# PalamaraLab/FastSMC

Measured on NVIDIA B200. Metric: hmm_pair_sites_per_s, higher is better.
Workload: dtype f32

## Files before the change

fastsmc_b200/csrc/decode_fast.cuh:

```cuda
#pragma once

#include "decode_kernels.cuh"

namespace fsmc
{

constexpr int kMaxParamStates = 160;

struct FastModel {
  DeviceModel base;
  float colRatios[kMaxParamStates];
  float expTimes[kMaxParamStates];
  float prior[kMaxParamStates];
};

__device__ __forceinline__ uint32_t smemPtr(const void* p)
{
  return static_cast<uint32_t>(__cvta_generic_to_shared(p));
}
__device__ __forceinline__ void mbarInit(uint64_t* bar, const uint32_t count)
{
  asm volatile("mbarrier.init.shared::cta.b64 [%0], %1;" ::"r"(smemPtr(bar)), "r"(count) : "memory");
}
__device__ __forceinline__ void mbarExpectTx(uint64_t* bar, const uint32_t bytes)
// ... 248 lines not shown
          const float2 t = __fmul2_rn(pk(f4(u4, 2 * jp), f4(u4, 2 * jp + 1)), xx);
          const float au0 = au;
          const float au1 = fmaf(colRatios[k], au0, t.x);
          au = fmaf(colRatios[k1], au1, t.y);
          const float2 tt = __ffma2_rn(pk(f4(d4, 2 * jp), f4(d4, 2 * jp + 1)), xx, pk(au0, au1));
          const float2 w = __fmul2_rn(pk(f4(e4, 2 * jp), f4(e4, 2 * jp + 1)),
                                      __ffma2_rn(pk(f4(b4, 2 * jp), f4(b4, 2 * jp + 1)), pk(y[k], y[k1]), tt));
          y[k] = w.x;
          y[k1] = w.y;
        } else if (k < S) {
          y[k] = f4(e4, 2 * jp) * fmaf(f4(d4, 2 * jp), x[k], au);
        }
      }
    }
    {
      const int ql = QM - 1 - i;
      const float4 e4 = E[ql], b4 = Br[ql];
#pragma unroll
      for (int jp = 1; jp >= 0; --jp) {
        const int k = 4 * ql + 2 * jp, k1 = k + 1;
        const float s1 = run;
        const float s0 = s1 + x[k1];
        run = s0 + x[k];
        const float2 w = __fmul2_rn(pk(f4(e4, 2 * jp), f4(e4, 2 * jp + 1)),
                                    __ffma2_rn(pk(f4(b4, 2 * jp), f4(b4, 2 * jp + 1)), pk(s0, s1), pk(y[k], y[k1])));
        y[k] = w.x;
        y[k1] = w.y;
      }
    }
  }
  return run;
}

template <int S>
__device__ __forceinline__ void backwardStepFolded(const float (&x)[S], float (&y)[S], const float* row, const int cls)
{
  constexpr int SQ = (S + 3) / 4, Spad = SQ * 4, QM = (SQ + 1) / 2;
  static_assert(4 * QM < S - 1, "the lower half lies below the last state");
  const float4* UsE = reinterpret_cast<const float4*>(row + cls * Spad);
  const float4* DE = reinterpret_cast<const float4*>(row + (3 + cls) * Spad);
  const float4* BE = reinterpret_cast<const float4*>(row + (6 + cls) * Spad);
  const float4* Rr = reinterpret_cast<const float4*>(row + 9 * Spad);
  float bu = 0.f, bl = 0.f;
  float above = 0.f;
#pragma unroll
  for (int i = 0; i < QM; ++i) {
    const int qu = SQ - 1 - i;
    if (qu >= QM) {
      const float4 u4 = UsE[qu], r4 = Rr[qu];
#pragma unroll
      for (int jp = 1; jp >= 0; --jp) {
        const int k = 4 * qu + 2 * jp, k1 = k + 1;
        if (k1 < S) {
          const float2 t = __fmul2_rn(pk(f4(u4, 2 * jp), f4(u4, 2 * jp + 1)), pk(x[k], x[k1]));
          if (k1 == S - 1) {
            y[k1] = 0.f;
          } else {
            bu = fmaf(f4(r4, 2 * jp + 1), bu, above);
            y[k1] = bu;
          }
          bu = fmaf(f4(r4, 2 * jp), bu, t.y);
          y[k] = bu;
          above = t.x;
        } else if (k < S) {
          above = f4(u4, 2 * jp) * x[k];
          if (k == S - 1) {
            y[k] = 0.f;
          } else {
            bu = fmaf(f4(r4, 2 * jp), bu, above);
            y[k] = bu;
          }
        }
      }
    }
    {
      const int ql = i;
      const float4 d4 = DE[ql], b4 = BE[ql];
#pragma unroll
      for (int jp = 0; jp < 2; ++jp) {
        const int k = 4 * ql + 2 * jp, k1 = k + 1;
        const float bl0 = bl;
        const float bl1 = fmaf(f4(b4, 2 * jp), x[k], bl0);
        bl = fmaf(f4(b4, 2 * jp + 1), x[k1], bl1);
        const float2 w = __ffma2_rn(pk(f4(d4, 2 * jp), f4(d4, 2 * jp + 1)), pk(x[k], x[k1]), pk(bl0, bl1));
        y[k] = w.x;
        y[k1] = w.y;
      }
    }
  }
#pragma unroll
  for (int i = 0; i < QM; ++i) {
    {
      const int ql = QM - 1 - i;
      const float4 u4 = UsE[ql], r4 = Rr[ql];
#pragma unroll
      for (int jp = 1; jp >= 0; --jp) {
        const int k = 4 * ql + 2 * jp, k1 = k + 1;
        const float2 t = __fmul2_rn(pk(f4(u4, 2 * jp), f4(u4, 2 * jp + 1)), pk(x[k], x[k1]));
        const float b1 = fmaf(f4(r4, 2 * jp + 1), bu, above);
        const float b0 = fmaf(f4(r4, 2 * jp), b1, t.y);
        bu = b0;
        above = t.x;
        const float2 w = __fadd2_rn(pk(y[k], y[k1]), pk(b0, b1));
        y[k] = w.x;
        y[k1] = w.y;
      }
    }
    const int qu = QM + i;
    if (qu < SQ) {
      const float4 d4 = DE[qu], b4 = BE[qu];
#pragma unroll
      for (int jp = 0; jp < 2; ++jp) {
        const int k = 4 * qu + 2 * jp, k1 = k + 1;
        if (k1 < S) {
          const float bl0 = bl;
          const float bl1 = fmaf(f4(b4, 2 * jp), x[k], bl0);
          bl = fmaf(f4(b4, 2 * jp + 1), x[k1], bl1);
          const float2 w = __fadd2_rn(__ffma2_rn(pk(f4(d4, 2 * jp), f4(d4, 2 * jp + 1)), pk(x[k], x[k1]), pk(bl0, bl1)),
                                      pk(y[k], y[k1]));
          y[k] = w.x;
          y[k1] = w.y;
        } else if (k < S) {
          y[k] = fmaf(f4(d4, 2 * jp), x[k], bl) + y[k];
        }
      }
    }
  }
}

static __device__ __noinline__ int emitSparseItems(SparseItem* items, float* itemAlpha, unsigned long long* itemCount,
                                            const long long capacity, const bool pred, const uint32_t pair, const int block,
                                            const int first, const int last, int chain, const float4* alphaStart,
                                            const int lane, const int SQ)
{
  const unsigned mask = __ballot_sync(kFull, pred);
  if (!mask) {
    return chain;
  }
  unsigned long long base = 0;
  if (lane == 0) {
    base = atomicAdd(itemCount, static_cast<unsigned long long>(__popc(mask)));
  }
  base = __shfl_sync(kFull, base, 0);
  if (pred) {
    const long long slot = static_cast<long long>(base) + __popc(mask & ((1u << lane) - 1u));
    if (slot < capacity) {
      items[slot] = SparseItem{pair, block, first, last, chain};
      float4* dst = reinterpret_cast<float4*>(itemAlpha + static_cast<size_t>(slot) * SQ * 4);
      for (int q = 0; q < SQ; ++q) {
        dst[q] = alphaStart[q * 32 + lane];
      }
    }
    chain = static_cast<int>(slot);
  }
  return chain;
}

constexpr int kNarrowMaxQuads = 4;
constexpr int kNarrowGroup = 4;

template <int S_T, int RQ, int G> struct NarrowSlot {
  static constexpr int SQ = (S_T + 3) / 4, Spad = SQ * 4;
  static constexpr uint32_t kCoefBytes = kBwdArrays * Spad * 4;
  static constexpr uint32_t kRecBytes = RQ * 32 * 16;
  static constexpr uint32_t kBytes = G * kCoefBytes + (G + 1) * kRecBytes;
};

template <int S_T, int RQ, int G, int DEPTH, int THREADS, int MIN_BLOCKS, int SPARSE_V = 0>
__global__ void __launch_bounds__(THREADS, MIN_BLOCKS) decodeNarrowKernel(const FastModel fm, const DecodeArgs args)
{
  constexpr bool SPARSE = (SPARSE_V & 1) != 0;
  constexpr bool kSkipFwd = (SPARSE_V & 2) != 0, kSkipBwd = (SPARSE_V & 4) != 0;
  constexpr int kGroupUnroll = (SPARSE_V & 64) ? G / 2 : 1;
  constexpr bool kSkipAlpha = (SPARSE_V & 8) != 0, kSkipBoundaryItems = (SPARSE_V & 16) != 0, kSkipRunItems = (SPARSE_V & 32) != 0;
  constexpr int S = S_T;
  constexpr int SQ = (S + 3) / 4;
  constexpr int Spad = SQ * 4;
  constexpr int NR = 4 * RQ - 1;
  using Slot = NarrowSlot<S_T, RQ, G>;
  constexpr uint32_t kRecBytes = Slot::kRecBytes;
  constexpr uint32_t kCoefBytes = Slot::kCoefBytes;
  constexpr size_t kRecFloats = static_cast<size_t>(RQ) * 32 * 4;
  constexpr size_t kRowFloats = static_cast<size_t>(kRowArrays) * Spad;
  constexpr uint32_t kRowBytes = static_cast<uint32_t>(kRowFloats) * 4;
  constexpr size_t kBwdFloats = static_cast<size_t>(kBwdArrays) * Spad;
  constexpr int kWarps = THREADS / 32;
  constexpr size_t kWarpBytes = static_cast<size_t>(DEPTH) * Slot::kBytes;
  static_assert(S >= 4 * kNarrowMaxQuads && RQ >= 1 && RQ <= kNarrowMaxQuads, "record quads index the state vector");
  static_assert(G % 2 == 0, "the two state vectors swap roles every step");

  extern __shared__ __align__(128) unsigned char smemRaw[];
  const DeviceModel m = fm.base;
  const int lane = threadIdx.x & 31;
  const int warp = threadIdx.x >> 5;
  unsigned char* mine = smemRaw + static_cast<size_t>(warp) * kWarpBytes;
  uint64_t* bars = reinterpret_cast<uint64_t*>(smemRaw + static_cast<size_t>(kWarps) * kWarpBytes) + warp * DEPTH;
  auto coefArea = [&](const int slot) { return reinterpret_cast<float*>(mine + static_cast<size_t>(slot) * Slot::kBytes); };
  auto recArea = [&](const int slot) {
    return reinterpret_cast<float4*>(mine + static_cast<size_t>(slot) * Slot::kBytes + static_cast<size_t>(G) * kCoefBytes);
  };
  if (lane == 0) {
    for (int i = 0; i < DEPTH; ++i) {
      mbarInit(&bars[i], 1);
    }
    asm volatile("fence.mbarrier_init.release.cluster;" ::: "memory");
  }
  __syncwarp();
  uint32_t parity = 0;

  const unsigned flags = args.flags;
  const bool wantSeg = flags & FSMC_CALL_SEGMENTS;
  const bool wantAge = !SPARSE && (flags & FSMC_SEG_AGE) && wantSeg;
  const int sT = m.stateThreshold;
  const long long warpGlobal = static_cast<long long>(blockIdx.x) * kWarps + warp;
  float* slab = args.scratch + warpGlobal * args.scratchPerWarp;
  constexpr size_t kVecFloats = static_cast<size_t>(SQ) * 32 * 4;
  const int ckShift = SPARSE ? args.ckptShift : 0;
  const int ckMask = (1 << ckShift) - 1;
  float4* alphaStart = SPARSE ? reinterpret_cast<float4*>(args.alphaScratch + warpGlobal * kVecFloats) : nullptr;

  for (;;) {
    unsigned long long t = 0;
    if (lane == 0) {
      t = atomicAdd(args.tileCounter, 1ull);
    }
    t = __shfl_sync(kFull, t, 0);
    if (static_cast<long long>(t) >= args.numTiles) {
      break;
    }
    const int tile = args.order ? args.order[t] : static_cast<int>(t);
    const int nPairs = args.tilePairs[tile];
    const int from = args.tileFrom[tile];
    const int len = args.tileTo[tile] - from;
    const int scanFrom = wantSeg ? args.tileScanFrom[tile] : 0;
    const int scanTo = wantSeg ? args.tileScanTo[tile] : 0;
    const bool laneActive = lane < nPairs;
    const int srcLane = laneActive ? lane : nPairs - 1;
    const uint32_t pair = static_cast<uint32_t>(tile) * 32u + static_cast<uint32_t>(lane);
    PairBits bits;
    bits.a = m.haps + static_cast<size_t>(args.hapA[static_cast<size_t>(tile) * 32 + srcLane]) * m.wordsPerHap;
    bits.b = m.haps + static_cast<size_t>(args.hapB[static_cast<size_t>(tile) * 32 + srcLane]) * m.wordsPerHap;
    const float* rowBase = m.siteRows + static_cast<size_t>(from) * kRowFloats;
    const long long ckptSlot0 = SPARSE ? args.tileCkptBase[tile] : 0;
    auto storeVector = [&](const float (&v)[S], float4* dst) {
#pragma unroll
      for (int q = 0; q < SQ; ++q) {
        dst[q * 32 + lane] = make_float4(v[4 * q], 4 * q + 1 < S ? v[4 * q + 1] : 0.f, 4 * q + 2 < S ? v[4 * q + 2] : 0.f,
                                         4 * q + 3 < S ? v[4 * q + 3] : 0.f);
      }
    };
    auto storeCheckpoint = [&](const float (&v)[S], const int p) {
      storeVector(v, reinterpret_cast<float4*>(args.ckptBeta + static_cast<size_t>(ckptSlot0 + (p >> ckShift)) * kVecFloats));
    };

    float a[S], c[S];
    float acc[NR];
#pragma unroll
    for (int k = 0; k < NR; ++k) {
      acc[k] = 0.f;
    }

    auto stageRecord = [&](const float (&v)[S], float4* out, const float divisor) {
#pragma unroll
      for (int q = 0; q < RQ; ++q) {
        float w[4];
#pragma unroll
        for (int i = 0; i < 4; ++i) {
          const int k = 4 * q + i;
          w[i] = k == NR ? divisor : (k < sT ? v[k] : 0.f);
        }
        out[q * 32 + lane] = make_float4(w[0], w[1], w[2], w[3]);
      }
    };

    {
      const int steps = len - 1;
      const int first = SPARSE ? min(steps, (len % G) ? (len % G) : G) : G;
      const int nGroups = steps <= 0 ? 0 : 1 + (max(steps - first, 0) + G - 1) / G;
      auto groupBegin = [&](const int g) { return g == 0 ? 0 : first + (g - 1) * G; };
      auto prefetch = [&](const int g) {
        if (lane == 0) {
          const int j0 = groupBegin(g), j1 = min(steps, j0 + (g == 0 ? first : G));
          const int slot = g % DEPTH;
          const uint32_t bytes = static_cast<uint32_t>(j1 - j0) * kCoefBytes;
          mbarExpectTx(&bars[slot], bytes);
          bulkLoad(coefArea(slot), m.bwdRows + static_cast<size_t>(from + len - j1) * kBwdFloats, bytes, &bars[slot]);
        }
      };
      for (int g = 0; g < DEPTH && g < nGroups; ++g) {
        prefetch(g);
      }
#pragma unroll
      for (int k = 0; k < S; ++k) {
        a[k] = 1.f;
      }
      if constexpr (SPARSE) {
        storeCheckpoint(a, len - 1);
      }
      if (nGroups == 0) {
        stageRecord(a, recArea(0), 1.0f);
        fenceProxyAsync();
        __syncwarp();
        if (lane == 0) {
          bulkStore(slab, recArea(0), kRecBytes);
          bulkCommit();
        }
      }
      for (int g = 0; g < nGroups; ++g) {
        const int slot = g % DEPTH;
        const int j0 = groupBegin(g);
        const int n = min(g == 0 ? first : G, steps - j0);
        const float* coef = coefArea(slot);
        float4* stage = recArea(slot);
        if constexpr (SPARSE && !kSkipBwd) {
          if (g > 0 && ((len - 1 - j0) & ckMask) == ckMask) {
            storeCheckpoint(a, len - 1 - j0);
          }
        }
        if (lane == 0) {
          bulkWaitRead<DEPTH - 1>();
        }
        mbarWait(&bars[slot], (parity >> slot) & 1u);
        parity ^= 1u << slot;
        __syncwarp();
        if (g == 0) {
          stageRecord(a, stage + static_cast<size_t>(n) * RQ * 32, 1.0f);
        }
        auto step = [&](const int i, float (&x)[S], float (&y)[S], const bool rescale) {
          const int p = len - 2 - (j0 + i);
          const int cls = bits.cls(from + p + 1);
          backwardStepFolded<S>(x, y, coef + static_cast<size_t>(n - 1 - i) * kBwdFloats, cls);
          float divisor = 1.0f;
          if (rescale) {
            divisor = sumStates<S>(y);
            scaleStates<S>(y, 1.0f / divisor);
          }
          stageRecord(y, stage + static_cast<size_t>(n - 1 - i) * RQ * 32, divisor);
        };
#pragma unroll(kGroupUnroll)
        for (int i = 0; i < G; i += 2) {
          if (i < n) {
            step(i, a, c, false);
          }
          if (i + 1 < n) {
            step(i + 1, c, a, i + 1 == G - 1);
          }
        }
        fenceProxyAsync();
        __syncwarp();
        if (lane == 0) {
          const int j1 = j0 + n;
          bulkStore(slab + static_cast<size_t>(len - 1 - j1) * kRecFloats, stage,
                    static_cast<uint32_t>(n + (g == 0 ? 1 : 0)) * kRecBytes);
          bulkCommit();
        }
        if (g + DEPTH < nGroups) {
          prefetch(g + DEPTH);
        }
        if (SPARSE && g == 0 && (n & 1)) {
#pragma unroll
          for (int k = 0; k < S; ++k) {
            a[k] = c[k];
          }
        }
      }
      const int rest = SPARSE ? max(steps - first, 0) : steps;
      if (rest & 1) {
      } else {
#pragma unroll
        for (int k = 0; k < S; ++k) {
          c[k] = a[k];
        }
      }
      if (lane == 0) {
        bulkWaitAll<0>();
      }
      __syncwarp();
    }

    {
      const int nGroups = (len + G - 1) / G;
      auto prefetch = [&](const int g) {
        if (lane == 0) {
          const int p0 = g * G;
          const uint32_t n = static_cast<uint32_t>(min(G, len - p0));
          const int slot = g % DEPTH;
          mbarExpectTx(&bars[slot], n * (kRowBytes + kRecBytes));
          bulkLoad(coefArea(slot), rowBase + static_cast<size_t>(p0) * kRowFloats, n * kRowBytes, &bars[slot]);
          bulkLoad(recArea(slot), slab + static_cast<size_t>(p0) * kRecFloats, n * kRecBytes, &bars[slot]);
        }
      };
      for (int g = 0; g < DEPTH && g < nGroups; ++g) {
        prefetch(g);
      }
      CallerState cs;
      float Z = 1.f, bPrev = 1.f;
      bool runOpen = false;
      int pieceStart = 0, chain = -1;
      auto emitItems = [&](const bool pred, const int block, const int first, const int last) {
        chain = emitSparseItems(args.items, args.itemAlpha, args.itemCount, args.itemCapacity, pred, pair, block, first, last, chain,
                                alphaStart, lane, SQ);
      };

      auto consume = [&](const int p, const float (&v)[S], float4* rec) {
        const int site = from + p;
        float q[4 * RQ];
#pragma unroll
        for (int qq = 0; qq < RQ; ++qq) {
          const float4 r4 = rec[qq * 32 + lane];
#pragma unroll
          for (int i = 0; i < 4; ++i) {
            q[4 * qq + i] = f4(r4, i);
          }
        }
        bPrev = q[NR];
        float ibdRaw = 0.f;
#pragma unroll
        for (int k = 0; k < NR; ++k) {
          q[k] *= v[k];
          ibdRaw += q[k];
        }
        const float r = 1.0f / Z;
        const float ibd = ibdRaw * r;
        if ((flags & FSMC_SITE_IBD) && laneActive) {
          args.siteIbd[static_cast<size_t>(pair) * args.siteStride + p] = ibd;
        }
        const bool inScan = wantSeg && site >= scanFrom && site < scanTo;
        if (inScan) {
          int now = ibd >= m.thr[0] ? 0 : (ibd >= m.thr[1] ? 1 : (ibd >= m.thr[2] ? 2 : (ibd >= m.thr[3] ? 3 : -1)));
          if (!laneActive) {
            now = -1;
          }
          const bool changed = now != cs.level;
          const bool ending = changed && cs.level >= 0;
          const bool closing = now >= 0 && site == scanTo - 1;
          const float rr = now >= 0 ? r : 0.f;
          const float keep = changed ? 0.f : 1.f;
          if constexpr (SPARSE && !kSkipFwd) {
            if (__any_sync(kFull, ending || closing)) {
              if constexpr (!kSkipRunItems) {
                emitItems(ending && runOpen && pieceStart <= site - 1, (p - 1) >> ckShift, pieceStart, site - 1);
              }
              if (ending) {
                emitSegment<false>(m, args, pair, cs.start, site - 1, cs.prob, cs.level, nullptr, false, chain);
                chain = -1;
                runOpen = false;
              }
              if (now >= 0 && changed) {
                runOpen = true;
                pieceStart = site;
              }
              if constexpr (!kSkipRunItems) {
                emitItems(closing, p >> ckShift, pieceStart, site);
              }
              if (closing) {
                emitSegment<false>(m, args, pair, changed ? site : cs.start, site, changed ? ibd : cs.prob + ibd, now, nullptr,
                                   false, chain);
                chain = -1;
                runOpen = false;
              }
            } else if (now >= 0 && changed) {
              runOpen = true;
              pieceStart = site;
            }
          } else if (__any_sync(kFull, ending || closing)) {
            float* park = reinterpret_cast<float*>(rec) + lane;
            __syncwarp();
            if (wantAge) {
#pragma unroll
              for (int k = 0; k < NR; ++k) {
                park[k * 32] = acc[k];
              }
              __syncwarp();
            }
            if (ending) {
              emitSegment<false>(m, args, pair, cs.start, site - 1, cs.prob, cs.level, park, wantAge);
            }
            __syncwarp();
            if (wantAge) {
#pragma unroll
              for (int k = 0; k < NR; ++k) {
                acc[k] = fmaf(q[k], rr, keep * acc[k]);
                park[k * 32] = acc[k];
              }
              __syncwarp();
            }
            if (closing) {
              emitSegment<false>(m, args, pair, changed ? site : cs.start, site, changed ? ibd : cs.prob + ibd, now, park, wantAge);
            }
            __syncwarp();
          } else if (wantAge) {
#pragma unroll
            for (int k = 0; k < NR; ++k) {
              acc[k] = fmaf(q[k], rr, keep * acc[k]);
            }
          }
          cs.prob = (now >= 0 && !closing) ? (changed ? ibd : cs.prob + ibd) : 0.f;
          cs.start = (now >= 0 && changed) ? site : cs.start;
          cs.level = now;
        }
      };

      for (int g = 0; g < nGroups; ++g) {
        const int slot = g % DEPTH;
        const int p0 = g * G;
        const int n = min(G, len - p0);
        const float* coef = coefArea(slot);
        float4* recs = recArea(slot);
        mbarWait(&bars[slot], (parity >> slot) & 1u);
        parity ^= 1u << slot;
        if constexpr (SPARSE && !kSkipFwd) {
          if (g > 0 && (p0 & ckMask) == 0) {
            if constexpr (!kSkipBoundaryItems) {
              if (__any_sync(kFull, runOpen)) {
                emitItems(runOpen, (p0 - 1) >> ckShift, pieceStart, from + p0 - 1);
              }
            }
            pieceStart = from + p0;
            if constexpr (!kSkipAlpha) {
              storeVector(c, alphaStart);
            }
          }
        }
        auto step = [&](const int i, float (&x)[S], float (&y)[S], const bool rescale) {
          const int p = p0 + i;
          const int cls = bits.cls(from + p);
          const float total = forwardStep<S>(fm.colRatios, x, y, coef + static_cast<size_t>(i) * kRowFloats, cls);
          float sc = 1.0f;
          if (rescale) {
            sc = 1.0f / total;
            scaleStates<S>(y, sc);
          }
          Z *= bPrev * sc;
          consume(p, y, recs + static_cast<size_t>(i) * RQ * 32);
        };
#pragma unroll(kGroupUnroll)
        for (int i = 0; i < G; i += 2) {
          if (i == 0 && g == 0) {
            const int cls = bits.cls(from);
            const float4* E = reinterpret_cast<const float4*>(coef + cls * Spad);
            float z0 = 0.f, z1 = 0.f, z2 = 0.f, z3 = 0.f;
#pragma unroll
            for (int q = 0; q < SQ; ++q) {
              const float4 e4 = E[q];
#pragma unroll
              for (int j = 0; j < 4; ++j) {
                const int k = 4 * q + j;
                if (k < S) {
                  a[k] = fm.prior[k] * f4(e4, j);
                }
              }
              z0 = fmaf(a[4 * q], c[4 * q], z0);
              if (4 * q + 1 < S) z1 = fmaf(a[4 * q + 1], c[4 * q + 1], z1);
              if (4 * q + 2 < S) z2 = fmaf(a[4 * q + 2], c[4 * q + 2], z2);
              if (4 * q + 3 < S) z3 = fmaf(a[4 * q + 3], c[4 * q + 3], z3);
            }
            Z = (z0 + z1) + (z2 + z3);
            consume(0, a, recs);
          } else if (i < n) {
            step(i, c, a, false);
          }
          if (i + 1 < n) {
            step(i + 1, a, c, i + 1 == G - 1);
          }
        }
        __syncwarp();
        if (g + DEPTH < nGroups) {
          prefetch(g + DEPTH);
        }
      }
    }
    __syncwarp();
  }
}

template <int S_T, int DEPTH, int RESCALE, bool ACC, int THREADS, int MIN_BLOCKS, bool SUM = false>
__global__ void __launch_bounds__(THREADS, MIN_BLOCKS) decodeFastKernel(const FastModel fm, const DecodeArgs args)
{
  constexpr int S = S_T;
  constexpr int SQ = (S + 3) / 4;
  constexpr int Spad = SQ * 4;
  constexpr uint32_t kBetaBytes = SQ * 32 * 16;
  constexpr uint32_t kCoefBytes = kRowArrays * Spad * 4;
  constexpr size_t kBetaFloats = static_cast<size_t>(SQ) * 32 * 4;
  constexpr int kWarps = THREADS / 32;
  constexpr size_t kWarpBytes = static_cast<size_t>(DEPTH) * (kBetaBytes + kCoefBytes);

  extern __shared__ __align__(128) unsigned char smemRaw[];
  const DeviceModel m = fm.base;
  const int lane = threadIdx.x & 31;
  const int warp = threadIdx.x >> 5;
  unsigned char* mine = smemRaw + static_cast<size_t>(warp) * kWarpBytes;
  uint64_t* bars = reinterpret_cast<uint64_t*>(smemRaw + static_cast<size_t>(kWarps) * kWarpBytes) +
                   warp * 2 * DEPTH;
  auto betaSlot = [&](const int i) { return reinterpret_cast<float4*>(mine + static_cast<size_t>(i) * kBetaBytes); };
  auto coefSlot = [&](const int i) {
    return reinterpret_cast<const float*>(mine + static_cast<size_t>(DEPTH) * kBetaBytes + static_cast<size_t>(i) * kCoefBytes);
  };
  if (lane == 0) {
    for (int i = 0; i < 2 * DEPTH; ++i) {
      mbarInit(&bars[i], 1);
    }
    asm volatile("fence.mbarrier_init.release.cluster;" ::: "memory");
  }
  __syncwarp();
  uint32_t betaParity = 0, coefParity = 0;

  const unsigned flags = args.flags;
  const bool wantSeg = flags & FSMC_CALL_SEGMENTS;
  const bool wantAge = ACC && (flags & FSMC_SEG_AGE) && wantSeg;
  const bool wantSite = flags & (FSMC_SITE_MEAN | FSMC_SITE_MAP);
  const int sT = m.stateThreshold;
  const int nAcc = m.ageThreshold;
  const long long warpGlobal = static_cast<long long>(blockIdx.x) * kWarps + warp;
  float* slab = args.scratch + warpGlobal * args.scratchPerWarp;
  const int sumPlanes = SUM && (flags & FSMC_SUM_BY_GENOTYPE) ? 3 : 1;
  float* sumMine = SUM ? args.sumScratch + static_cast<size_t>(warpGlobal) * sumPlanes * m.L * Spad : nullptr;
  const long long totalWarps = static_cast<long long>(gridDim.x) * kWarps;

  for (long long turn = 0;; ++turn) {
    unsigned long long t = 0;
    if constexpr (SUM) {
      t = static_cast<unsigned long long>(warpGlobal + turn * totalWarps);
    } else {
      if (lane == 0) {
        t = atomicAdd(args.tileCounter, 1ull);
      }
      t = __shfl_sync(kFull, t, 0);
    }
    if (static_cast<long long>(t) >= args.numTiles) {
      break;
    }
    const int tile = args.order ? args.order[t] : static_cast<int>(t);
    const int nPairs = args.tilePairs[tile];
    const int from = args.tileFrom[tile];
    const int len = args.tileTo[tile] - from;
    const int scanFrom = wantSeg ? args.tileScanFrom[tile] : 0;
    const int scanTo = wantSeg ? args.tileScanTo[tile] : 0;
    const bool laneActive = lane < nPairs;
    const int srcLane = laneActive ? lane : nPairs - 1;
    const uint32_t pair = static_cast<uint32_t>(tile) * 32u + static_cast<uint32_t>(lane);
    PairBits bits;
    bits.a = m.haps + static_cast<size_t>(args.hapA[static_cast<size_t>(tile) * 32 + srcLane]) * m.wordsPerHap;
    bits.b = m.haps + static_cast<size_t>(args.hapB[static_cast<size_t>(tile) * 32 + srcLane]) * m.wordsPerHap;
    const float* rowBase = m.siteRows + static_cast<size_t>(from) * kRowArrays * Spad;

    float a[S], c[S];
    float acc[ACC ? S : 1];
#pragma unroll
    for (int k = 0; k < (ACC ? S : 1); ++k) {
      acc[k] = 0.f;
    }

    auto storeRow = [&](const float (&v)[S], const int p, const int bslot) {
      if (lane == 0) {
        bulkWaitRead<DEPTH - 1>();
      }
      __syncwarp();
      float4* out = betaSlot(bslot);
#pragma unroll
      for (int q = 0; q < SQ; ++q) {
        out[q * 32 + lane] = make_float4(v[4 * q], 4 * q + 1 < S ? v[4 * q + 1] : 0.f, 4 * q + 2 < S ? v[4 * q + 2] : 0.f,
                                         4 * q + 3 < S ? v[4 * q + 3] : 0.f);
      }
      fenceProxyAsync();
      __syncwarp();
      if (lane == 0) {
        bulkStore(slab + static_cast<size_t>(p) * kBetaFloats, out, kBetaBytes);
        bulkCommit();
      }
    };

    {
      auto prefetchCoef = [&](const int j) {
        if (lane == 0) {
          uint64_t* bar = &bars[DEPTH + j % DEPTH];
          mbarExpectTx(bar, kCoefBytes);
          bulkLoad(const_cast<float*>(coefSlot(j % DEPTH)), rowBase + static_cast<size_t>(len - 1 - j) * kRowArrays * Spad,
                   kCoefBytes, bar);
        }
      };
      const int steps = len - 1;
      for (int j = 0; j < DEPTH && j < steps; ++j) {
        prefetchCoef(j);
      }
#pragma unroll
      for (int k = 0; k < S; ++k) {
        a[k] = 1.f;
      }
      storeRow(a, len - 1, 0);
      auto step = [&](const int j, float (&x)[S], float (&y)[S]) {
        const int p = len - 2 - j;
        const int slot = j % DEPTH;
        const int cls = bits.cls(from + p + 1);
        mbarWait(&bars[DEPTH + slot], (coefParity >> slot) & 1u);
        coefParity ^= 1u << slot;
        backwardStep<S>(x, y, coefSlot(slot), cls);
        __syncwarp();
        if (j + DEPTH < steps) {
          prefetchCoef(j + DEPTH);
        }
        if ((p & (RESCALE - 1)) == 0) {
          scaleStates<S>(y, 1.0f / sumStates<S>(y));
        }
        storeRow(y, p, (j + 1) % DEPTH);
      };
      int j = 0;
      for (; j + 1 < steps; j += 2) {
        step(j, a, c);
        step(j + 1, c, a);
      }
      if (j < steps) {
        step(j, a, c);
      }
      if (lane == 0) {
        bulkWaitAll<0>();
      }
// ... 249 lines not shown
```

fastsmc_b200/csrc/decode_kernels.cuh:

```cuda
#pragma once

#include <cstdint>
#include <cuda_runtime.h>

#include "../../include/fastsmc_b200.h"

namespace fsmc
{

constexpr int kRowArrays = 8;
constexpr int kBwdArrays = 10;
constexpr unsigned kFull = 0xffffffffu;

struct DeviceModel {
  int S;
  int Spad;
  int L;
  const float* siteRows;
  const float* bwdRows;
  const float* laneAux;
  const float* prior;
  const float* expTimes;
  const float* colRatios;
  int stateThreshold;
  int ageThreshold;
  float thr[4];
  const uint64_t* haps;
  long long wordsPerHap;
};

struct SparseItem {
  uint32_t pair;
  int32_t block;
  int32_t first, last;
  int32_t prev;
};

struct DecodeArgs {
  const uint32_t* hapA;
  const uint32_t* hapB;
  const int* tilePairs;
  const int* tileFrom;
  const int* tileTo;
  const int* tileScanFrom;
  const int* tileScanTo;
  const int* order;
  long long numTiles;
  unsigned flags;
  fsmc_segment* segments;
  unsigned long long* segmentCount;
  long long segmentCapacity;
  float* siteMean;
  int* siteMap;
  float* siteIbd;
  long long siteStride;
  float* sitePosterior;
  float* sumPosterior;
  float* scratch;
  long long scratchPerWarp;
  float* accScratch;
  unsigned long long* tileCounter;
  int ckptShift;
  const long long* tileCkptBase;
  float* ckptBeta;
  float* alphaScratch;
  SparseItem* items;
  float* itemAlpha;
  float* itemSums;
  unsigned long long* itemCount;
  long long itemCapacity;
  const uint32_t* itemOrder;
  unsigned long long* refineCounter;
  float* sumScratch;
};

template <bool EXACT> __device__ __forceinline__ float mulAdd(float a, float b, float c)
{
  if constexpr (EXACT) {
    return __fadd_rn(__fmul_rn(a, b), c);
  } else {
    return fmaf(a, b, c);
  }
}
template <bool EXACT> __device__ __forceinline__ float mulMulAdd(float a, float b, float c, float d)
{
  if constexpr (EXACT) {
    return __fadd_rn(__fmul_rn(a, b), __fmul_rn(c, d));
  } else {
    return fmaf(a, b, c * d);
  }
}

template <int N> struct RegVec {
  float v[N];
  __device__ __forceinline__ float get(int k) const { return v[k]; }
  __device__ __forceinline__ void set(int k, float x) { v[k] = x; }
};
struct SmemVec {
  float* p;
  __device__ __forceinline__ float get(int k) const { return p[k * 32]; }
  __device__ __forceinline__ void set(int k, float x) { p[k * 32] = x; }
};

__device__ __forceinline__ float4 ldg4(const float* p)
{
  return __ldg(reinterpret_cast<const float4*>(p));
}
__device__ __forceinline__ float elem(const float4& v, int j)
{
  return j == 0 ? v.x : (j == 1 ? v.y : (j == 2 ? v.z : v.w));
}

template <int S_T, class F> __device__ __forceinline__ void forStatesBelow(const int limit, F&& f)
{
  if constexpr (S_T > 0) {
#pragma unroll
    for (int g = 0; g < (S_T + 7) / 8; ++g) {
      if (8 * g < limit) {
#pragma unroll
        for (int j = 0; j < 8; ++j) {
          const int k = 8 * g + j;
          if (k < S_T && k < limit) {
            f(k);
          }
        }
      }
    }
  } else {
    for (int k = 0; k < limit; ++k) {
      f(k);
    }
  }
}

struct PairBits {
  const uint64_t* a;
  const uint64_t* b;
  uint64_t x = 0, t = 0;
  long long word = -1;
  __device__ __forceinline__ int cls(int site)
  {
    const long long w = site >> 6;
    if (w != word) {
      const uint64_t wa = __ldg(a + w), wb = __ldg(b + w);
      x = wa ^ wb;
      t = wa & wb;
      word = w;
    }
    const int bit = site & 63;
    return ((x >> bit) & 1ull) ? 1 : (((t >> bit) & 1ull) ? 2 : 0);
  }
};

template <int S_T, bool EXACT, class VecA, class VecC>
__device__ __forceinline__ void sweepBackward(const DeviceModel& m, PairBits& bits, const int from, const int len,
                                              VecA& b, VecC& c, float* __restrict__ beta )
{
  const int S = S_T ? S_T : m.S;
  const int SQ = (S_T ? (S_T + 3) / 4 : m.Spad / 4);
  const int Spad = SQ * 4;
  const size_t plane = static_cast<size_t>(S) * 32;

  {
    float sum = 0.f;
#pragma unroll
    for (int k = 0; k < S; ++k) {
      sum = __fadd_rn(sum, 1.0f);
    }
    const float sc = 1.0f / sum;
    float* out = beta + static_cast<size_t>(len - 1) * plane;
#pragma unroll
    for (int k = 0; k < S; ++k) {
      const float v = __fmul_rn(1.0f, sc);
      b.set(k, v);
      out[k * 32] = v;
    }
  }

  for (int p = len - 2; p >= 0; --p) {
    const int site = from + p + 1;
    const float* row = m.siteRows + static_cast<size_t>(site) * kRowArrays * Spad;
    const float* E = row + bits.cls(site) * Spad;
    const float* Dr = row + 3 * Spad;
    const float* Br = row + 4 * Spad;
    const float* Ur = row + 5 * Spad;
    const float* Rr = row + 6 * Spad;

#pragma unroll
    for (int q = 0; q < SQ; ++q) {
      const float4 e4 = ldg4(E + 4 * q);
#pragma unroll
      for (int j = 0; j < 4; ++j) {
        const int k = 4 * q + j;
        if (k < S) {
          b.set(k, __fmul_rn(b.get(k), elem(e4, j)));
        }
      }
    }
    {
      float bu = 0.f;
#pragma unroll
      for (int q = SQ - 1; q >= 0; --q) {
        const float4 u4 = ldg4(Ur + 4 * q);
        const float4 r4 = ldg4(Rr + 4 * q);
#pragma unroll
        for (int j = 3; j >= 0; --j) {
          const int k = 4 * q + j;
          if (k == S - 1) {
            c.set(k, 0.f);
          } else if (k < S - 1) {
            bu = mulMulAdd<EXACT>(elem(u4, j), b.get(k + 1), elem(r4, j), bu);
            c.set(k, bu);
          }
        }
      }
    }
    float sum = 0.f;
    {
      float bl = 0.f, bPrev = 0.f, vPrev = 0.f;
#pragma unroll
      for (int q = 0; q < SQ; ++q) {
        const float4 d4 = ldg4(Dr + 4 * q);
        const float4 b4 = ldg4(Br + 4 * q);
#pragma unroll
        for (int j = 0; j < 4; ++j) {
          const int k = 4 * q + j;
          if (k < S) {
            const float v = b.get(k);
            if (k) {
              bl = mulAdd<EXACT>(bPrev, vPrev, bl);
            }
            const float nb = __fadd_rn(mulAdd<EXACT>(elem(d4, j), v, bl), c.get(k));
            c.set(k, nb);
            sum = __fadd_rn(sum, nb);
            bPrev = elem(b4, j);
            vPrev = v;
          }
        }
      }
    }
    const float sc = 1.0f / sum;
    float* out = beta + static_cast<size_t>(p) * plane;
#pragma unroll
    for (int k = 0; k < S; ++k) {
      const float v = __fmul_rn(c.get(k), sc);
      b.set(k, v);
      out[k * 32] = v;
    }
  }
}

template <bool EXACT>
__device__ __noinline__ void emitSegment(const DeviceModel& m, const DecodeArgs& a, const uint32_t pair, const int start,
                                         const int end, const float prob, const int level,
                                         const float* acc , const bool age,
                                         const int lastItem = -1 )
{
  fsmc_segment s;
  s.pair = pair;
  s.posStart = start;
  s.posEnd = end;
  s.prob = prob;
  s.level = level;
  s.postMean = 0.f;
  s.mapTime = 0.f;
  s.mapState = lastItem;
  if (age) {
    const int n = m.ageThreshold;
    float tot = 0.f;
    for (int k = 0; k < n; ++k) {
      tot = __fadd_rn(tot, acc[k * 32]);
    }
    const float norm = 1.f / tot;
    float mean = 0.f;
    int best = 0;
    float bestRatio = acc[0] / __ldg(m.prior);
    for (int k = 0; k < n; ++k) {
      const float x = acc[k * 32];
      mean = __fadd_rn(mean, __fmul_rn(__fmul_rn(norm, x), __ldg(m.expTimes + k)));
      const float r = x / __ldg(m.prior + k);
      if (bestRatio < r) {
        bestRatio = r;
        best = k;
      }
    }
    s.postMean = mean;
    s.mapState = best;
    s.mapTime = __ldg(m.expTimes + best);
  }
  const unsigned long long idx = atomicAdd(a.segmentCount, 1ull);
  if (static_cast<long long>(idx) < a.segmentCapacity) {
    a.segments[idx] = s;
  }
}

struct CallerState {
  int level = -1;
  int start = 0;
  float prob = 0.f;
};

template <int S_T, bool EXACT, class VecA, class VecC>
__device__ __forceinline__ void sweepForward(const DeviceModel& m, const DecodeArgs& args, PairBits& bits,
                                             const int from, const int len, const int scanFrom, const int scanTo,
                                             const uint32_t pair, const bool laneActive, VecA& a, VecC& c,
                                             const float* __restrict__ beta, float* acc )
// ... 315 lines not shown
```

Measured before the change: 17.72 billion.

## Defer segment emission to per-group replay and preload genotype bits per group

The forward decode loop no longer runs warp votes and segment or sparse-item emission inline at each site. It records per-lane event state into a spare shared-memory area, sets a bitmask of event sites, and replays those events after each group in a separate noinline function. Per-site classification now reads bits preloaded once per group into a 32-bit window instead of checking the cached word at every site. The intent is to keep the inner recurrence branch-free and free of warp divergence. In exchange, every site now pays extra shared-memory stores for event data and the parked accumulators, plus a function-call replay path.

```diff
diff --git a/fastsmc_b200/csrc/decode_fast.cuh b/fastsmc_b200/csrc/decode_fast.cuh
--- a/fastsmc_b200/csrc/decode_fast.cuh
+++ b/fastsmc_b200/csrc/decode_fast.cuh
@@ -424,6 +424,69 @@
       }
     }
     chain = static_cast<int>(slot);
+  }
+  return chain;
+}
+
+constexpr int kEvEnding = 1 << 6, kEvClosing = 1 << 7, kEvChanged = 1 << 8, kEvRunItem = 1 << 9;
+template <bool SPARSE>
+static __device__ __noinline__ int replayGroupEvents(const DeviceModel& m, const DecodeArgs& args, const uint32_t pair,
+                                                     const int lane, const unsigned evMask, const int site0, const int p0,
+                                                     const int n, const float4* ev, const float4* recs, const int RQ,
+                                                     const int G, float* park, const bool wantAge, const bool runItems,
+                                                     int chain, const int ckShift, const float4* alphaStart, const int SQ)
+{
+  __syncwarp();
+  const int NR = 4 * RQ - 1;
+  auto unpark = [&](const int j) {
+    for (int k = 0; k < NR; ++k) {
+      park[k * 32 + lane] = f4(recs[(static_cast<size_t>(j) * RQ + (k >> 2)) * 32 + lane], k & 3);
+    }
+  };
+  for (int i = 0; i < n; ++i) {
+    const bool evt = (evMask >> i) & 1u;
+    if (!__any_sync(kFull, evt)) {
+      continue;
+    }
+    const int site = site0 + i, p = p0 + i;
+    const float4 e = ev[i * 32 + lane];
+    const int bits = evt ? __float_as_int(e.w) : 0;
+    const int start = __float_as_int(e.x);
+    const float prob = e.y, ibd = e.z;
+    const int levelOld = (bits & 7) - 1, now = ((bits >> 3) & 7) - 1;
+    const bool ending = bits & kEvEnding, closing = bits & kEvClosing, changed = bits & kEvChanged;
+    if constexpr (SPARSE) {
+      const int pieceStart = __float_as_int(recs[static_cast<size_t>(i) * RQ * 32 + lane].x);
+      if (runItems) {
+        chain = emitSparseItems(args.items, args.itemAlpha, args.itemCount, args.itemCapacity, (bits & kEvRunItem) != 0, pair,
+                                (p - 1) >> ckShift, pieceStart, site - 1, chain, alphaStart, lane, SQ);
+      }
+      if (ending) {
+        emitSegment<false>(m, args, pair, start, site - 1, prob, levelOld, nullptr, false, chain);
+        chain = -1;
+      }
+      if (runItems) {
+        chain = emitSparseItems(args.items, args.itemAlpha, args.itemCount, args.itemCapacity, closing, pair, p >> ckShift,
+                                (now >= 0 && changed) ? site : pieceStart, site, chain, alphaStart, lane, SQ);
+      }
+      if (closing) {
+        emitSegment<false>(m, args, pair, changed ? site : start, site, changed ? ibd : prob + ibd, now, nullptr, false, chain);
+        chain = -1;
+      }
+    } else {
+      if (ending) {
+        if (wantAge) {
+          unpark(i == 0 ? G : i - 1);
+        }
+        emitSegment<false>(m, args, pair, start, site - 1, prob, levelOld, park + lane, wantAge);
+      }
+      if (closing) {
+        if (wantAge) {
+          unpark(i);
+        }
+        emitSegment<false>(m, args, pair, changed ? site : start, site, changed ? ibd : prob + ibd, now, park + lane, wantAge);
+      }
+    }
   }
   return chain;
 }
@@ -509,7 +572,7 @@
     const bool laneActive = lane < nPairs;
     const int srcLane = laneActive ? lane : nPairs - 1;
     const uint32_t pair = static_cast<uint32_t>(tile) * 32u + static_cast<uint32_t>(lane);
-    PairBits bits;
+    GroupBits bits;
     bits.a = m.haps + static_cast<size_t>(args.hapA[static_cast<size_t>(tile) * 32 + srcLane]) * m.wordsPerHap;
     bits.b = m.haps + static_cast<size_t>(args.hapB[static_cast<size_t>(tile) * 32 + srcLane]) * m.wordsPerHap;
     const float* rowBase = m.siteRows + static_cast<size_t>(from) * kRowFloats;
@@ -584,6 +647,7 @@
         const int n = min(g == 0 ? first : G, steps - j0);
         const float* coef = coefArea(slot);
         float4* stage = recArea(slot);
+        bits.load(from + len - j0 - n, n);
         if constexpr (SPARSE && !kSkipBwd) {
           if (g > 0 && ((len - 1 - j0) & ckMask) == ckMask) {
             storeCheckpoint(a, len - 1 - j0);
@@ -674,15 +738,25 @@
                                 alphaStart, lane, SQ);
       };
 
-      auto consume = [&](const int p, const float (&v)[S], float4* rec) {
+      static_assert(G * (kBwdFloats - kRowFloats) >= static_cast<size_t>(G) * 32 * 4, "one float4 per lane and site");
+      auto evArea = [&](const int slot) { return reinterpret_cast<float4*>(coefArea(slot) + G * kRowFloats); };
+      unsigned evMask = 0;
+      auto parkAcc = [&](float4* rec) {
+#pragma unroll
+        for (int qq = 0; qq < RQ; ++qq) {
+          rec[qq * 32 + lane] = make_float4(acc[4 * qq], acc[4 * qq + 1], acc[4 * qq + 2], 4 * qq + 3 < NR ? acc[4 * qq + 3] : 0.f);
+        }
+      };
+
+      auto consume = [&](const int i, const int p, const float (&v)[S], float4* rec, float4* ev) {
         const int site = from + p;
         float q[4 * RQ];
 #pragma unroll
         for (int qq = 0; qq < RQ; ++qq) {
           const float4 r4 = rec[qq * 32 + lane];
 #pragma unroll
-          for (int i = 0; i < 4; ++i) {
-            q[4 * qq + i] = f4(r4, i);
+          for (int j = 0; j < 4; ++j) {
+            q[4 * qq + j] = f4(r4, j);
           }
         }
         bPrev = q[NR];
@@ -698,79 +772,41 @@
           args.siteIbd[static_cast<size_t>(pair) * args.siteStride + p] = ibd;
         }
         const bool inScan = wantSeg && site >= scanFrom && site < scanTo;
-        if (inScan) {
-          int now = ibd >= m.thr[0] ? 0 : (ibd >= m.thr[1] ? 1 : (ibd >= m.thr[2] ? 2 : (ibd >= m.thr[3] ? 3 : -1)));
-          if (!laneActive) {
-            now = -1;
-          }
-          const bool changed = now != cs.level;
-          const bool ending = changed && cs.level >= 0;
-          const bool closing = now >= 0 && site == scanTo - 1;
+        int now = ibd >= m.thr[3] ? 3 : -1;
+        now = ibd >= m.thr[2] ? 2 : now;
+        now = ibd >= m.thr[1] ? 1 : now;
+        now = ibd >= m.thr[0] ? 0 : now;
+        now = laneActive ? now : -1;
+        const bool changed = inScan && now != cs.level;
+        const bool ending = changed && cs.level >= 0;
+        const bool closing = inScan && now >= 0 && site == scanTo - 1;
+        const bool starting = changed && now >= 0;
+        const bool event = ending || closing;
+        const bool runItem = SPARSE & ending & runOpen & (pieceStart <= site - 1);
+        const int packed = (cs.level + 1) | ((now + 1) << 3) | (ending ? kEvEnding : 0) | (closing ? kEvClosing : 0) |
+                           (changed ? kEvChanged : 0) | (runItem ? kEvRunItem : 0);
+        ev[lane] = make_float4(__int_as_float(cs.start), cs.prob, ibd, __int_as_float(packed));
+        evMask |= event ? 1u << i : 0u;
+        if constexpr (SPARSE) {
+          rec[lane].x = __int_as_float(pieceStart);
+          runOpen = !closing && (starting || (!ending && runOpen));
+          pieceStart = starting ? site : pieceStart;
+        } else {
           const float rr = now >= 0 ? r : 0.f;
           const float keep = changed ? 0.f : 1.f;
-          if constexpr (SPARSE && !kSkipFwd) {
-            if (__any_sync(kFull, ending || closing)) {
-              if constexpr (!kSkipRunItems) {
-                emitItems(ending && runOpen && pieceStart <= site - 1, (p - 1) >> ckShift, pieceStart, site - 1);
-              }
-              if (ending) {
-                emitSegment<false>(m, args, pair, cs.start, site - 1, cs.prob, cs.level, nullptr, false, chain);
-                chain = -1;
-                runOpen = false;
-              }
-              if (now >= 0 && changed) {
-                runOpen = true;
-                pieceStart = site;
-              }
-              if constexpr (!kSkipRunItems) {
-                emitItems(closing, p >> ckShift, pieceStart, site);
-              }
-              if (closing) {
-                emitSegment<false>(m, args, pair, changed ? site : cs.start, site, changed ? ibd : cs.prob + ibd, now, nullptr,
-                                   false, chain);
-                chain = -1;
-                runOpen = false;
-              }
-            } else if (now >= 0 && changed) {
-              runOpen = true;
-              pieceStart = site;
-            }
-          } else if (__any_sync(kFull, ending || closing)) {
-            float* park = reinterpret_cast<float*>(rec) + lane;
-            __syncwarp();
-            if (wantAge) {
-#pragma unroll
-              for (int k = 0; k < NR; ++k) {
-                park[k * 32] = acc[k];
-              }
-              __syncwarp();
-            }
-            if (ending) {
-              emitSegment<false>(m, args, pair, cs.start, site - 1, cs.prob, cs.level, park, wantAge);
-            }
-            __syncwarp();
-            if (wantAge) {
-#pragma unroll
-              for (int k = 0; k < NR; ++k) {
-                acc[k] = fmaf(q[k], rr, keep * acc[k]);
-                park[k * 32] = acc[k];
-              }
-              __syncwarp();
-            }
-            if (closing) {
-              emitSegment<false>(m, args, pair, changed ? site : cs.start, site, changed ? ibd : cs.prob + ibd, now, park, wantAge);
-            }
-            __syncwarp();
-          } else if (wantAge) {
-#pragma unroll
-            for (int k = 0; k < NR; ++k) {
-              acc[k] = fmaf(q[k], rr, keep * acc[k]);
-            }
-          }
-          cs.prob = (now >= 0 && !closing) ? (changed ? ibd : cs.prob + ibd) : 0.f;
-          cs.start = (now >= 0 && changed) ? site : cs.start;
-          cs.level = now;
-        }
+#pragma unroll
+          for (int k = 0; k < NR; ++k) {
+            acc[k] = inScan ? fmaf(q[k], rr, keep * acc[k]) : acc[k];
+          }
+          if (wantAge) {
+            parkAcc(rec);
+          }
+        }
+        const float grown = cs.prob + ibd;
+        const float prob = (now >= 0 && !closing) ? (changed ? ibd : grown) : 0.f;
+        cs.prob = inScan ? prob : cs.prob;
+        cs.start = starting ? site : cs.start;
+        cs.level = inScan ? now : cs.level;
       };
 
       for (int g = 0; g < nGroups; ++g) {
@@ -779,8 +815,13 @@
         const int n = min(G, len - p0);
         const float* coef = coefArea(slot);
         float4* recs = recArea(slot);
+        float4* ev = evArea(slot);
+        bits.load(from + p0, n);
         mbarWait(&bars[slot], (parity >> slot) & 1u);
         parity ^= 1u << slot;
+        if (!SPARSE && wantAge) {
+          parkAcc(recs + static_cast<size_t>(G) * RQ * 32);
+        }
         if constexpr (SPARSE && !kSkipFwd) {
           if (g > 0 && (p0 & ckMask) == 0) {
             if constexpr (!kSkipBoundaryItems) {
@@ -804,37 +845,44 @@
             scaleStates<S>(y, sc);
           }
           Z *= bPrev * sc;
-          consume(p, y, recs + static_cast<size_t>(i) * RQ * 32);
+          consume(i, p, y, recs + static_cast<size_t>(i) * RQ * 32, ev + i * 32);
         };
+        if (g == 0) {
+          const int cls = bits.cls(from);
+          const float4* E = reinterpret_cast<const float4*>(coef + cls * Spad);
+          float z0 = 0.f, z1 = 0.f, z2 = 0.f, z3 = 0.f;
+#pragma unroll
+          for (int q = 0; q < SQ; ++q) {
+            const float4 e4 = E[q];
+#pragma unroll
+            for (int j = 0; j < 4; ++j) {
+              const int k = 4 * q + j;
+              if (k < S) {
+                a[k] = fm.prior[k] * f4(e4, j);
+              }
+            }
+            z0 = fmaf(a[4 * q], c[4 * q], z0);
+            if (4 * q + 1 < S) z1 = fmaf(a[4 * q + 1], c[4 * q + 1], z1);
+            if (4 * q + 2 < S) z2 = fmaf(a[4 * q + 2], c[4 * q + 2], z2);
+            if (4 * q + 3 < S) z3 = fmaf(a[4 * q + 3], c[4 * q + 3], z3);
+          }
+          Z = (z0 + z1) + (z2 + z3);
+          consume(0, 0, a, recs, ev);
+        }
 #pragma unroll(kGroupUnroll)
         for (int i = 0; i < G; i += 2) {
-          if (i == 0 && g == 0) {
-            const int cls = bits.cls(from);
-            const float4* E = reinterpret_cast<const float4*>(coef + cls * Spad);
-            float z0 = 0.f, z1 = 0.f, z2 = 0.f, z3 = 0.f;
-#pragma unroll
-            for (int q = 0; q < SQ; ++q) {
-              const float4 e4 = E[q];
-#pragma unroll
-              for (int j = 0; j < 4; ++j) {
-                const int k = 4 * q + j;
-                if (k < S) {
-                  a[k] = fm.prior[k] * f4(e4, j);
-                }
-              }
-              z0 = fmaf(a[4 * q], c[4 * q], z0);
-              if (4 * q + 1 < S) z1 = fmaf(a[4 * q + 1], c[4 * q + 1], z1);
-              if (4 * q + 2 < S) z2 = fmaf(a[4 * q + 2], c[4 * q + 2], z2);
-              if (4 * q + 3 < S) z3 = fmaf(a[4 * q + 3], c[4 * q + 3], z3);
-            }
-            Z = (z0 + z1) + (z2 + z3);
-            consume(0, a, recs);
-          } else if (i < n) {
+          if (i < n && (i | g) != 0) {
             step(i, c, a, false);
           }
           if (i + 1 < n) {
             step(i + 1, a, c, i + 1 == G - 1);
           }
+        }
+        if (__any_sync(kFull, evMask != 0)) {
+          chain = replayGroupEvents<SPARSE>(m, args, pair, lane, evMask, from + p0, p0, n, ev, recs, RQ, G,
+                                            coefArea(slot), wantAge, !kSkipFwd && !kSkipRunItems, chain, ckShift,
+                                            alphaStart, SQ);
+          evMask = 0;
         }
         __syncwarp();
         if (g + DEPTH < nGroups) {
diff --git a/fastsmc_b200/csrc/decode_kernels.cuh b/fastsmc_b200/csrc/decode_kernels.cuh
--- a/fastsmc_b200/csrc/decode_kernels.cuh
+++ b/fastsmc_b200/csrc/decode_kernels.cuh
@@ -152,6 +152,32 @@
   }
 };
 
+struct GroupBits {
+  const uint64_t* a;
+  const uint64_t* b;
+  uint32_t x = 0, t = 0;
+  int base = 0;
+  __device__ __forceinline__ void load(const int lo, const int n)
+  {
+    const int w0 = lo >> 6, w1 = (lo + n - 1) >> 6, sh = lo & 63;
+    const uint64_t a0 = __ldg(a + w0), b0 = __ldg(b + w0);
+    uint64_t xx = (a0 ^ b0) >> sh, tt = (a0 & b0) >> sh;
+    if (w1 != w0) {
+      const uint64_t a1 = __ldg(a + w1), b1 = __ldg(b + w1);
+      xx |= (a1 ^ b1) << (64 - sh);
+      tt |= (a1 & b1) << (64 - sh);
+    }
+    x = static_cast<uint32_t>(xx);
+    t = static_cast<uint32_t>(tt);
+    base = lo;
+  }
+  __device__ __forceinline__ int cls(const int site) const
+  {
+    const int bit = site - base;
+    return ((x >> bit) & 1u) ? 1 : (((t >> bit) & 1u) ? 2 : 0);
+  }
+};
+
 template <int S_T, bool EXACT, class VecA, class VecC>
 __device__ __forceinline__ void sweepBackward(const DeviceModel& m, PairBits& bits, const int from, const int len,
                                               VecA& b, VecC& c, float* __restrict__ beta )
```

New measurement: 17.94 billion (median of 6 runs). 1.2% higher.
